# bruAristimunha/Synthetic-Sleep-EEG-Signal-Generation-using-Latent-Diffusion-Models

Hardware: AMD Instinct MI355X
Metric: EEG windows/sec (LDM train step) (higher is better)
Workload: dtype bf16; 1 GPU; LDM train step on raw (B,1,3072) windows: frozen AutoencoderKL[32,32,64] encode+sample x scale, add_noise, config_ldm.yaml UNet (30.5M params, latent_channels=1) fwd+bwd, epsilon MSE, Adam lr 1e-4 [BASELINE configs[2]/[3]: per-GPU batch 256 = global 2048 / 8]; per_gpu_batch=256, global_batch=256, latent_len=768, parallelism=dp1

## Files before the change

### synthetic-sleep-eeg-signal-generation-using-latent-diffusion-models_amd/csrc/gemm.hip

```cpp
#include <stdlib.h>
#include <string.h>

#include "common.h"

namespace {


template <typename T> struct Tr;
template <> struct Tr<float> { static constexpr int KC = 16; static constexpr int EPC = 4; };
template <> struct Tr<bf16_t> { static constexpr int KC = 32; static constexpr int EPC = 8; };
template <> struct Tr<f16_t> { static constexpr int KC = 32; static constexpr int EPC = 8; };

template <typename T> __device__ __forceinline__ void mma(const uint4& a, const uint4& b, f32x4& acc);
template <> __device__ __forceinline__ void mma<float>(const uint4& a, const uint4& b, f32x4& acc) {
  acc = __builtin_amdgcn_mfma_f32_16x16x4f32(__uint_as_float(a.x), __uint_as_float(b.x), acc, 0, 0, 0);
  acc = __builtin_amdgcn_mfma_f32_16x16x4f32(__uint_as_float(a.y), __uint_as_float(b.y), acc, 0, 0, 0);
  acc = __builtin_amdgcn_mfma_f32_16x16x4f32(__uint_as_float(a.z), __uint_as_float(b.z), acc, 0, 0, 0);
  acc = __builtin_amdgcn_mfma_f32_16x16x4f32(__uint_as_float(a.w), __uint_as_float(b.w), acc, 0, 0, 0);
}
template <> __device__ __forceinline__ void mma<bf16_t>(const uint4& a, const uint4& b, f32x4& acc) {
  acc = __builtin_amdgcn_mfma_f32_16x16x32_bf16(__builtin_bit_cast(bf16x8, a), __builtin_bit_cast(bf16x8, b), acc, 0, 0, 0);
}

template <> __device__ __forceinline__ void mma<f16_t>(const uint4& a, const uint4& b, f32x4& acc) {
  acc = __builtin_amdgcn_mfma_f32_16x16x32_f16(__builtin_bit_cast(f16x8, a), __builtin_bit_cast(f16x8, b), acc, 0, 0, 0);
}

typedef s16x4 __attribute__((address_space(3))) * lds_s16x4_ptr;

template <int KSUB> __device__ __forceinline__ int nt_swz(int row, int slot) {
  if constexpr (KSUB == 1) return slot ^ (((row >> 2) & 1) * 3);
  else return slot ^ (2 * ((row >> 1) & 3));
}
template <int BX> __device__ __forceinline__ int tr_swz(int row, int colbyte) {
  constexpr int WIN = ((BX * 2) & (BX * 2 - 1)) == 0 ? BX * 2 - 1 : 127;
  static_assert((BX * 2) % (WIN + 1) == 0, "TR rows must be whole swizzle windows");
  return colbyte ^ ((((row & 3) | (((row >> 3) & 1) << 2)) * 32) & WIN);
}

template <typename T, int BX> struct TrPitch;
template <int BX> struct TrPitch<float, BX> { static constexpr int v = BX * 4 + 16; };
template <int BX> struct TrPitch<bf16_t, BX> { static constexpr int v = BX * 2; };
template <int BX> struct TrPitch<f16_t, BX> { static constexpr int v = BX * 2; };

template <int BX>
__device__ __forceinline__ uint4 read_tr_f32(const char* tile, int ks, int x0, int lm, int q, int rowoff) {
  constexpr int pitch = TrPitch<float, BX>::v;
  const char* p = tile + (ks * 16 + 4 * q + rowoff) * pitch + (x0 + lm) * 4;
  uint4 r;
  r.x = *(const unsigned*)(p);
  r.y = *(const unsigned*)(p + pitch);
  r.z = *(const unsigned*)(p + 2 * pitch);
  r.w = *(const unsigned*)(p + 3 * pitch);
  return r;
}
template <int BX>
__device__ __forceinline__ uint4 read_tr_bf16(const char* tile, int ks, int x0, int lm, int q, int rowoff) {
  constexpr int pitch = TrPitch<bf16_t, BX>::v;
  const int row0 = ks * 32 + 8 * q + (lm >> 2) + rowoff, colb = (x0 + 4 * (lm & 3)) * 2;
  const char* p0 = tile + row0 * pitch + tr_swz<BX>(row0, colb);
  const char* p1 = tile + (row0 + 4) * pitch + tr_swz<BX>(row0 + 4, colb);
  s16x4 lo = __builtin_amdgcn_ds_read_tr16_b64_v4i16((lds_s16x4_ptr)(p0));
  s16x4 hi = __builtin_amdgcn_ds_read_tr16_b64_v4i16((lds_s16x4_ptr)(p1));
  uint4 r;
  r.x = (unsigned)(unsigned short)lo[0] | ((unsigned)(unsigned short)lo[1] << 16);
  r.y = (unsigned)(unsigned short)lo[2] | ((unsigned)(unsigned short)lo[3] << 16);
  r.z = (unsigned)(unsigned short)hi[0] | ((unsigned)(unsigned short)hi[1] << 16);
  r.w = (unsigned)(unsigned short)hi[2] | ((unsigned)(unsigned short)hi[3] << 16);
  return r;
}
template <typename T, int BX>
__device__ __forceinline__ uint4 read_tr_t(const char* tile, int ks, int x0, int lm, int q, int rowoff = 0) {
  if constexpr (sizeof(T) == 4) return read_tr_f32<BX>(tile, ks, x0, lm, q, rowoff);
  else return read_tr_bf16<BX>(tile, ks, x0, lm, q, rowoff);
}
template <typename T, int BX>
__device__ __forceinline__ int tr_store_off(int krow, int seg) {
  if constexpr (sizeof(T) == 4) return krow * TrPitch<float, BX>::v + seg * 16;
  else return krow * TrPitch<bf16_t, BX>::v + tr_swz<BX>(krow, seg * 16);
}

template <typename T, int AMODE, int BMODE, int TAPS, int KSUB, int BN, int STRIDE, int WMT, bool DMA>
struct Cfg {
  static constexpr int WM = (WMT == 3 || WMT == 6) ? 2 : (WMT == 5 ? 4 : WMT);
  static constexpr int FM = (WMT == 3) ? 6 : (WMT == 5 ? 2 : 4);
  static constexpr int BM = WM * FM * 16;
// ... 841 lines not shown
      const float4 v = *(const float4*)(ws + (long)r * n + i);
      s.x += v.x; s.y += v.y; s.z += v.z; s.w += v.w;
    }
  }
  if (ty > 0) red[ty - 1][tx] = s;
  __syncthreads();
  if (ty == 0 && ok) {
    float4 d = *(const float4*)(dst + i);
#pragma unroll
    for (int k = 0; k < 3; k++) { const float4 v = red[k][tx]; s.x += v.x; s.y += v.y; s.z += v.z; s.w += v.w; }
    d.x += s.x; d.y += s.y; d.z += s.z; d.w += s.w;
    *(float4*)(dst + i) = d;
  }
}

__global__ __launch_bounds__(256) void splitk_fold_grouped_kernel(const float* __restrict__ ws, int nsplit, long n, const GemmGroup* __restrict__ grp) {
  __shared__ float4 red[3][64];
  const int tx = threadIdx.x & 63, ty = threadIdx.x >> 6;
  const long i = ((long)blockIdx.x * 64 + tx) * 4;
  const bool ok = i < n;
  const float* w = ws + (long)blockIdx.y * nsplit * n;
  float4 s = make_float4(0.f, 0.f, 0.f, 0.f);
  if (ok) {
    for (int r = ty; r < nsplit; r += 4) {
      const float4 v = *(const float4*)(w + (long)r * n + i);
      s.x += v.x; s.y += v.y; s.z += v.z; s.w += v.w;
    }
  }
  if (ty > 0) red[ty - 1][tx] = s;
  __syncthreads();
  if (ty == 0 && ok) {
    float* dp = grp->Dst[blockIdx.y] + i;
    float4 d = *(const float4*)dp;
#pragma unroll
    for (int k = 0; k < 3; k++) { const float4 v = red[k][tx]; s.x += v.x; s.y += v.y; s.z += v.z; s.w += v.w; }
    d.x += s.x; d.y += s.y; d.z += s.z; d.w += s.w;
    *(float4*)dp = d;
  }
}

int gemm_launch_grouped(eegldm_ctx* ctx, const GemmArgs& a_in, const GemmGroup& g, int slot) {
  GemmArgs a = a_in;
  EEG_CHECK(slot >= 0 && slot < 4096, "group slot");
  if (slot >= ctx->grp_cap) {
    HIP_TRY(hipStreamSynchronize(ctx->stream)); if (ctx->side_on) HIP_TRY(hipStreamSynchronize(ctx->side));
    const int cap = slot + 64;
    GemmGroup* nd = nullptr; HIP_TRY(hipMalloc(&nd, sizeof(GemmGroup) * cap));
    if (ctx->grp_dev) { HIP_TRY(hipMemcpy(nd, ctx->grp_dev, sizeof(GemmGroup) * ctx->grp_cap, hipMemcpyDeviceToDevice)); HIP_TRY(hipFree(ctx->grp_dev)); }
    ctx->grp_dev = nd; ctx->grp_cap = cap; ctx->grp_host.resize(cap);
  }
  if ((int)ctx->grp_host.size() < ctx->grp_cap) ctx->grp_host.resize(ctx->grp_cap);
  if (memcmp(&ctx->grp_host[slot], &g, sizeof(GemmGroup)) != 0) {
    HIP_TRY(hipStreamSynchronize(ctx->stream)); if (ctx->side_on) HIP_TRY(hipStreamSynchronize(ctx->side));
    HIP_TRY(hipMemcpy(ctx->grp_dev + slot, &g, sizeof(GemmGroup), hipMemcpyHostToDevice));
    ctx->grp_host[slot] = g;
  }
  a.grp = ctx->grp_dev + slot;
  EEG_CHECK(a.ngroup >= 1 && a.ngroup <= GEMM_MAX_GROUP && a.amode == GA_TR && a.bmode == GB_TR && a.ztaps == 1 && (a.taps == 1 || a.taps == 3), "not a groupable weight gradient");
  const int epc = a.dtype == EEGLDM_F32 ? 4 : 8;
  EEG_CHECK(a.M % epc == 0 && a.N % epc == 0 && a.N % 4 == 0, "operand alignment");
  for (int i = 0; i < a.ngroup; i++) EEG_CHECK(g.lda[i] % epc == 0 && g.ldb[i] % epc == 0 && g.A[i] && g.B[i] && g.Dst[i], "group member %d: leading dimension / null pointer", i);
  if (a.splitk < 1) a.splitk = 1;
  a.batch = a.ngroup; a.out_f32 = 1; a.ups = 1; a.rows_per_vec = 1; a.ldc = a.N; a.sCt = (long)a.M * a.N; a.colsum = nullptr;
  const long fold_n = (long)a.taps * a.M * a.N;
  const int KST = 2 * (a.dtype == EEGLDM_F32 ? 16 : 32);
  int per = (a.K + a.splitk - 1) / a.splitk; per = (per + KST - 1) / KST * KST;
  a.splitk = (a.K + per - 1) / per;
  const size_t need = (size_t)a.ngroup * a.splitk * fold_n * sizeof(float);
  if (ctx->splitk_ws_bytes < need) {
    if (ctx->splitk_ws) { HIP_TRY(hipStreamSynchronize(ctx->stream)); if (ctx->side_on) HIP_TRY(hipStreamSynchronize(ctx->side)); HIP_TRY(hipFree(ctx->splitk_ws)); ctx->splitk_ws = nullptr; ctx->splitk_ws_bytes = 0; }
    HIP_TRY(hipMalloc(&ctx->splitk_ws, need)); ctx->splitk_ws_bytes = need;
  }
  a.C = ctx->splitk_ws; a.sCk = fold_n; a.sCb = (long)a.splitk * fold_n; a.atomic_out = 0; a.k_skew = 0.f;
  a.zero_page = ctx->zero_page;
  a.xcd_swizzle = 1;
  ProfRec rec; const bool prof = ctx->prof_on;
  if (prof) {
    rec.cls = a.taps == 3 ? PROF_CONV_WGRAD : PROF_GEMM_TN;
    rec.flops = 2.0 * a.M * a.N * (double)a.K * a.taps * a.ngroup;
    rec.M = a.M; rec.N = a.N; rec.K = a.K; rec.taps = a.taps; rec.splitk = a.splitk; rec.kern = "gemm_grouped";
    HIP_TRY(hipEventCreate(&rec.a)); HIP_TRY(hipEventCreate(&rec.b));
    HIP_TRY(hipEventRecord(rec.a, ctx->stream));
  }
  int rc;
  if (a.dtype == EEGLDM_F32) rc = launch_modes<float>(ctx, a);
  else if (a.dtype == EEGLDM_BF16) rc = launch_modes<bf16_t>(ctx, a);
  else if (a.dtype == EEGLDM_F16) rc = launch_modes<f16_t>(ctx, a);
  else EEG_FAIL(EEGLDM_ERR_UNSUPPORTED, "dtype %d", a.dtype);
  if (rc == 0) {
    hipLaunchKernelGGL(splitk_fold_grouped_kernel, dim3((unsigned)((fold_n / 4 + 63) / 64), a.ngroup), dim3(256), 0, ctx->stream, (const float*)ctx->splitk_ws, a.splitk, fold_n, a.grp);
    LAUNCH_CHECK();
  }
  if (prof) { HIP_TRY(hipEventRecord(rec.b, ctx->stream)); ctx->prof.push_back(rec); }
  return rc;
}

int gemm_launch(eegldm_ctx* ctx, const GemmArgs& a_in) {
  GemmArgs a = a_in;
  if (a.splitk < 1) a.splitk = 1;
  if (a.ztaps < 1) a.ztaps = 1;
  if (a.ups < 1) a.ups = 1;
  if (a.batch < 1) a.batch = 1;
  if (a.rows_per_vec < 1) a.rows_per_vec = 1;
  const int epc = a.dtype == EEGLDM_F32 ? 4 : 8;
  EEG_CHECK(a.M > 0 && a.N > 0 && a.K > 0, "empty problem M=%d N=%d K=%d", a.M, a.N, a.K);
  if (a.amode == GA_TR) EEG_CHECK(a.M % epc == 0 && a.lda % epc == 0, "A(TR): M, lda must be multiples of %d", epc);
  else EEG_CHECK(a.K % epc == 0 && a.lda % epc == 0, "A: K, lda must be multiples of %d (K=%d lda=%ld)", epc, a.K, a.lda);
  if (a.bmode == GB_TR) EEG_CHECK(a.N % epc == 0 && a.ldb % epc == 0, "B(TR): N, ldb must be multiples of %d", epc);
  else EEG_CHECK(a.K % epc == 0 && a.ldb % epc == 0, "B: K, ldb must be multiples of %d", epc);
  EEG_CHECK(!(a.atomic_out || a.splitk > 1) || a.out_f32, "atomic / split-K output must be f32");
  EEG_CHECK(a.N % 4 == 0 && a.ldc % 4 == 0, "N and ldc must be multiples of 4 (vector epilogue): N=%d ldc=%ld", a.N, a.ldc);
  EEG_CHECK(!a.resid || a.ldr % 4 == 0, "ldr must be a multiple of 4");
  EEG_CHECK(!a.rowvec || a.ld_rowvec % 4 == 0, "ld_rowvec must be a multiple of 4");
  EEG_CHECK(!a.colsum || (a.amode == GA_TR && a.dtype != EEGLDM_F32 && a.batch == 1), "fused column sums need a 16-bit transposed A operand and batch 1");
  float* fold_dst = nullptr; long fold_n = 0;
  constexpr bool fused_ws = true;
  const bool det_zt = eeg_deterministic() && a.ztaps > 1 && a.taps == 1 && a.sCt == (long)a.M * a.N;
  if (a.splitk > 1 && a.amode == GA_TR && a.bmode == GB_TR && (a.taps == 1 || (a.taps == 3 && a.sCt == (long)a.M * a.N && fused_ws)) && (a.ztaps == 1 || det_zt) && a.batch == 1 && a.atomic_out && a.ldc == a.N) {
    const size_t need = (size_t)a.splitk * a.taps * a.ztaps * a.M * a.N * sizeof(float);
    if (need <= (size_t)512 << 20) {
      if (ctx->splitk_ws_bytes < need) {
        if (ctx->splitk_ws) { HIP_TRY(hipStreamSynchronize(ctx->stream)); HIP_TRY(hipFree(ctx->splitk_ws)); ctx->splitk_ws = nullptr; ctx->splitk_ws_bytes = 0; }
        HIP_TRY(hipMalloc(&ctx->splitk_ws, need)); ctx->splitk_ws_bytes = need;
      }
      const int KST = 2 * (a.dtype == EEGLDM_F32 ? 16 : 32);
      int per = (a.K + a.splitk - 1) / a.splitk; per = (per + KST - 1) / KST * KST;
      a.splitk = (a.K + per - 1) / per;
      fold_dst = (float*)a.C; fold_n = (long)a.taps * a.ztaps * a.M * a.N;
      a.C = ctx->splitk_ws; a.sCk = fold_n; a.atomic_out = 0;
      if (det_zt) HIP_TRY(hipMemsetAsync(ctx->splitk_ws, 0, (size_t)a.splitk * fold_n * sizeof(float), ctx->stream));
    }
  }
  if (a.splitk > 1 && !fold_dst && eeg_deterministic()) a.splitk = 1;
  if (a.splitk > 1 && !fold_dst) a.atomic_out = 1;
  a.zero_page = ctx->zero_page;
  a.xcd_swizzle = 1;
  ProfRec rec; bool prof = ctx->prof_on;
  if (prof) {
    rec.cls = a.amode == GA_CONV ? (a.bmode == GB_NT ? PROF_CONV_FWD : PROF_CONV_DGRAD)
              : (a.amode == GA_TR ? ((a.conv_map || a.taps == 3) ? PROF_CONV_WGRAD : PROF_GEMM_TN) : (a.bmode == GB_NT ? PROF_GEMM_NT : PROF_GEMM_NN));
    rec.flops = 2.0 * a.M * a.N * (double)a.K * a.taps * a.ztaps * a.batch / (a.ups > 1 ? a.ups : 1);
    rec.M = a.M; rec.N = a.N; rec.K = a.K; rec.taps = a.taps * a.ztaps; rec.splitk = a.splitk;
    rec.kern = fold_dst ? "gemm_splitk_fold" : (a.b_kblk ? "gemm_kblk" : "gemm");
    HIP_TRY(hipEventCreate(&rec.a)); HIP_TRY(hipEventCreate(&rec.b));
    HIP_TRY(hipEventRecord(rec.a, ctx->stream));
  }
  a.k_skew = 0.f;
  if (a.splitk > 1 && a.amode == GA_TR && a.atomic_out && !fold_dst) {
    const int kst = (a.dtype == EEGLDM_F32 ? 16 : 32) * 2;
    const long S = ((long)a.K + kst - 1) / kst;
    const float spb = (float)S / (float)a.splitk;
    float sk = (66.0f - spb) / 84.0f;
    sk = sk < 0.f ? 0.f : (sk > 0.5f ? 0.5f : sk);
    if (sk > 0.f && spb * (1.0f - sk) >= 2.0f) a.k_skew = sk;
  }
  int rc = 0;
  if ((a.amode == GA_CONV || (a.amode == GA_PLAIN && a.taps == 1 && a.batch == 1)) && (a.dtype == EEGLDM_BF16 || a.dtype == EEGLDM_F16) && !fold_dst) {
    if (a.bmode == GB_NT) rc = gemm_big_try(ctx, a);
    else if (a.B_alt) { GemmArgs b = a; b.B = a.B_alt; b.bmode = GB_NT; b.b_kblk = 1; rc = gemm_big_try(ctx, b); }
    if (rc < 0) return rc;
  }
  if (rc == 1) { rc = 0; rec.kern = "gemm_big"; }
  else if (a.dtype == EEGLDM_F32) rc = launch_modes<float>(ctx, a);
  else if (a.dtype == EEGLDM_BF16) rc = launch_modes<bf16_t>(ctx, a);
  else if (a.dtype == EEGLDM_F16) rc = launch_modes<f16_t>(ctx, a);
  else EEG_FAIL(EEGLDM_ERR_UNSUPPORTED, "dtype %d", a.dtype);
  if (rc == 0 && fold_dst) {
    hipLaunchKernelGGL(splitk_fold_kernel, dim3((unsigned)((fold_n / 4 + 63) / 64)), dim3(256), 0, ctx->stream, (const float*)ctx->splitk_ws, a.splitk, fold_n, fold_dst);
    LAUNCH_CHECK();
  }
  if (prof) { HIP_TRY(hipEventRecord(rec.b, ctx->stream)); ctx->prof.push_back(rec); }
  return rc;
}
```

### synthetic-sleep-eeg-signal-generation-using-latent-diffusion-models_amd/csrc/internal.h

```cpp
#pragma once
#include "common.h"

int ew_temb(eegldm_ctx*, const int64_t* t, void* out, int B, int dim, int dtype);
int ew_silu(eegldm_ctx*, const float* x, void* y, long n, int dtype);
int ew_silu_bwd(eegldm_ctx*, const float* dy, const float* x, void* dx, long n, int dtype);
int eeg_det_buffer(eegldm_ctx*, size_t bytes, float** out);
int ew_fold_partials_det(eegldm_ctx*, const float* parts, int nparts, long stride, int off, int n, float* total);
int ew_colsum(eegldm_ctx*, const void* x, long ldx, float* out_ps, long ldo, float* total, int B, int L, int C, int dtype);
int ew_softmax(eegldm_ctx*, const float* S, void* P, long rows, int n, int dtype);
int ew_softmax_bwd(eegldm_ctx*, const float* dP, const void* P, void* dS, long rows, int n, float alpha, int dtype);
int ew_add_rows(eegldm_ctx*, void* dst, long ldd, const void* src, long lds, long rows, int C, int dtype);
int ew_dropout_rows(eegldm_ctx*, void* x, long ld, long rows, int C, float p, uint64_t seed, uint64_t offset, int dtype);
int ew_film_silu_fwd(eegldm_ctx*, const void* hn, long ldh, const float* emb, long lde, void* a, long lda, int B, int L, int C, int dtype);
int ew_film_silu_bwd(eegldm_ctx*, const void* hn, long ldh, const float* emb, long lde, const void* da, long ldda, void* dhn, long lddh,
                     float* demb, long ldde, int B, int L, int C, int dtype);
int ew_copy_rows(eegldm_ctx*, void* dst, long ldd, const void* src, long lds, long rows, int C, int dtype);

bool conv_is_thin(int Cin, int Cout, int dtype);
struct KbDesc { long off; long chunk0; int cout, cin; };
int kblk_pack(eegldm_ctx* ctx, const void* w_plain, void* w_packed, const KbDesc* d_table, int n, long total_chunks);
int kblk_pack_one(eegldm_ctx* ctx, const void* w_plain, void* w_packed, int Cout, int Cin, int taps = 3);
int kblk_pack_t(eegldm_ctx* ctx, const void* w_plain, void* w_packed, const KbDesc* d_table, int n, long total_chunks);
int kblk_pack_t_one(eegldm_ctx* ctx, const void* w_plain, void* w_packed, int Cout, int Cin, int taps = 3);
int s2ws_pack(eegldm_ctx* ctx, const void* w, void* wf, void* wd, int Cout, int Cin);
int dconv_run(eegldm_ctx*, int dtype, bool dgrad, const void* in, long ldin, const void* w, const float* bias,
              const void* resid, long ldr, void* out, long ldout, int B, int Lin, int Lout, int Cin, int Cout, int K,
              int stride, int pad_l, float act_slope = 0.f);
bool dconv_fuses_act(int dtype, int Cin, int Cout, int K, long ldout);
int dconv_wgrad(eegldm_ctx*, int dtype, const void* x, long ldx, const void* dy, long lddy, float* dw, int B, int Lin,
                int Lout, int Cin, int Cout, int K, int stride, int pad_l, float* dbias, int* bias_done);
bool dconv_wgrad_tinyv_ok(int Cin, int Cout, int K);

struct SkinnyGn { const float2* part; const float* gamma; const float* beta; int cpg; float eps; int silu;
                  const float2* part_b = nullptr; int nqa = 0; };
struct SkinnyExt { const void* x2; long ldx2; const void* w2; int Cin2; const float* bias2; };
bool conv_skinny_takes(int dtype, int Cin, int Cout, int taps, int B, int L);
int conv_skinny_ex(eegldm_ctx* ctx, int dtype, const void* x, long ldx, const void* w, int Cin, int Cout, int taps, const float* bias,
                   const float* rowvec, long ld_rowvec, const void* resid, long ldr, void* y, long ldy, int B, int L,
                   const SkinnyGn* gn, float2* part_out, const SkinnyExt* ext = nullptr);
int conv_skinny_try(eegldm_ctx* ctx, int dtype, const void* x, long ldx, const void* w, int Cin, int Cout, int taps, const float* bias,
                    const float* rowvec, long ld_rowvec, const void* resid, long ldr, void* y, long ldy, int B, int L);
int conv_ws2_try(eegldm_ctx*, int dtype, int dgrad, const void* x, const void* w, const float* bias, void* y, int B, int Lo,
                 float* col_parts = nullptr, int* col_nparts = nullptr);
int conv_ws_try(eegldm_ctx*, int dtype, const void* x, long ldx, const void* w, int Cin, int Cout, int transposed, const float* bias,
                const float* rowvec, long ld_rowvec, const void* resid, long ldr, void* y, long ldy, int B, int L,
                float* col_parts = nullptr, int* col_nparts = nullptr);

int op_conv_fwd(eegldm_ctx*, int dtype, const void* x, long ldx, const void* w, const float* bias, void* y, long ldy,
                int B, int Lin, int Cin, int Cout, int K, int stride, int pad_l, int pad_r,
                const float* rowvec, long ld_rowvec, const void* resid, long ldr, float act_slope = 0.f,
                float* col_parts = nullptr, int* col_nparts = nullptr);
bool op_conv_fuses_act(int dtype, int Cin, int Cout, int K, long ldy);
int op_conv3_skip_fwd(eegldm_ctx*, int dtype, const void* x, long ldx, const void* w, const float* bias, const void* x2, long ldx2,
                      const void* w2, const float* bias2, void* y, long ldy, int B, int L, int Cin, int Cin2, int Cout,
                      const float* rowvec, long ld_rowvec);
int op_conv_dgrad(eegldm_ctx*, int dtype, const void* dy, long lddy, const void* w, void* dx, long lddx,
                  int B, int Lin, int Cin, int Cout, int K, int stride, int pad_l, int pad_r, const void* resid, long ldr);
bool op_wgrad_fuses_bias(int dtype, int Cin, int Cout);
int op_gn_fold_flush(eegldm_ctx*);
int op_wgrad_flush(eegldm_ctx*);
int op_conv_wgrad(eegldm_ctx*, int dtype, const void* x, long ldx, const void* dy, long lddy, float* dw, float* dbias,
                  int B, int Lin, int Cin, int Cout, int K, int stride, int pad_l, int pad_r);
int op_linear(eegldm_ctx*, int dtype, const void* x, long ldx, const void* w, long ldw, const float* bias, void* y, long ldy,
              int M, int N, int K, int out_f32);
int op_linear_dgrad(eegldm_ctx*, int dtype, const void* dy, long lddy, const void* w, long ldw, void* dx, long lddx,
                    int M, int N, int K, int out_f32);
int op_linear_wgrad(eegldm_ctx*, int dtype, const void* x, long ldx, const void* dy, long lddy, float* dw, long lddw,
                    int M, int N, int K);
int op_attention_fwd(eegldm_ctx*, int dtype, const void* qkv, long ldq, void* out, long ldo, void* probs, float* logits,
                     int B, int T, int C);
int op_attention_bwd(eegldm_ctx*, int dtype, const void* qkv, long ldq, const void* probs, const void* dout, long lddo,
                     void* dqkv, long lddq, float* dprobs, void* dlogits, int B, int T, int C);
int op_groupnorm_bwd(eegldm_ctx*, const void* x, long ldx, const float* gamma, const float* beta, const float* stats,
                     const void* dy, long lddy, void* dx, long lddx, float* dgamma, float* dbeta, int B, int L, int C, int G,
                     int fuse_silu, int resample, const void* dxr, long lddxr, int dtype, float* colsum_ps, long ldps, int* colsum_done,
                     const void* dxr2 = nullptr, long lddxr2 = 0, int* dxr2_done = nullptr, int* slots_deferred = nullptr, int defer_region = 0);
int op_gn_slot_reduce_deferred(eegldm_ctx*, float* dgamma, float* dbeta, int C, int region = 0);
int ew_fold_partials(eegldm_ctx*, const float* parts, int nparts, int n, float* total);
bool pre_conv3_ok(int dtype, int Cin, int Cout, int L);
int pre_conv3_launch(eegldm_ctx*, const void* x, const double* in_stats, const float* gamma, const float* beta, const void* w,
                     const float* bias, const void* resid, void* y, double* out_stats, int B, int L, int Cin, int Cout, float eps, int dtype);
int sample_stats_launch(eegldm_ctx*, const void* x, long n_per_sample, int B, double* stats, int dtype);
bool attn_chain_ok(int dtype, int T, int C, long ldq, long ldo);
int attn_chain_fwd(eegldm_ctx*, const void* qkv, long ldq, void* out, long ldo, void* probs, int B, int T, int C, int dtype);
int attn_chain_bwd(eegldm_ctx*, const void* qkv, long ldq, const void* probs, const void* dout, long lddo, void* dq, long lddq,
                   void* dS, int B, int T, int C, int fuse_kv, int dtype);
bool attn_chain_bwd_fuses_kv(eegldm_ctx*, int B, int T);
```

### synthetic-sleep-eeg-signal-generation-using-latent-diffusion-models_amd/csrc/ops.hip

```cpp
#include <math.h>

#include "common.h"
#include "internal.h"
#include <string.h>

static inline int conv_lout(int Lin, int K, int stride, int pad_l, int pad_r) { return (Lin + pad_l + pad_r - K) / stride + 1; }

bool op_conv_fuses_act(int dtype, int Cin, int Cout, int K, long ldy) { return conv_is_thin(Cin, Cout, dtype) && dconv_fuses_act(dtype, Cin, Cout, K, ldy); }
int op_conv_fwd(eegldm_ctx* ctx, int dtype, const void* x, long ldx, const void* w, const float* bias, void* y, long ldy,
                int B, int Lin, int Cin, int Cout, int K, int stride, int pad_l, int pad_r,
                const float* rowvec, long ld_rowvec, const void* resid, long ldr, float act_slope, float* col_parts, int* col_nparts) {
  if (col_nparts) *col_nparts = 0;
  EEG_CHECK(B > 0 && Lin > 0 && Cin > 0 && Cout > 0 && (K == 1 || K == 3) && (stride == 1 || stride == 2),
            "unsupported conv B=%d Lin=%d Cin=%d Cout=%d K=%d stride=%d", B, Lin, Cin, Cout, K, stride);
  const int Lout = conv_lout(Lin, K, stride, pad_l, pad_r);
  EEG_CHECK(Lout > 0, "empty output");
  if (conv_is_thin(Cin, Cout, dtype)) {
    EEG_CHECK(rowvec == nullptr, "rowvec add is not available on the thin-channel path");
    return dconv_run(ctx, dtype, false, x, ldx, w, bias, resid, ldr, y, ldy, B, Lin, Lout, Cin, Cout, K, stride, pad_l, act_slope);
  }
  EEG_CHECK(act_slope <= 0.f, "fused activation is only available on the thin-input direct conv");
  if (K == 3 && stride == 2 && pad_l == 1 && pad_r == 1 && Cin == 64 && Cout == 128 && ldx == Cin && Lin == 2 * Lout && !rowvec && !resid &&
      dtype != EEGLDM_F32 && !ctx->s2ws_f.empty()) {
    auto it = ctx->s2ws_f.find(w);
// ... 88 lines not shown
    a.amode = GA_CONV; a.tap_flip = 1; a.Lout = Lin; a.Lin = Lin; a.stride = 1; a.pad_l = K - 1 - pad_l;
    a.ups = stride; a.Lsrc = Lout;
    if (dtype != EEGLDM_F32 && stride == 1 && !ctx->kblk_t.empty()) {
      auto it = ctx->kblk_t.find(w);
      if (it != ctx->kblk_t.end()) a.B_alt = it->second;
    }
  }
  return gemm_launch(ctx, a);
}

bool op_wgrad_fuses_bias(int dtype, int Cin, int Cout) {
  EEG_ENV_VAR(bool, fuse_bias, getenv("EEGLDM_NO_FUSED_BIAS_GRAD") == nullptr);
  if (!fuse_bias) return false;
  if (conv_is_thin(Cin, Cout, dtype)) return dconv_wgrad_tinyv_ok(Cin, Cout, 3);
  if (eeg_deterministic()) return false;
  return dtype != EEGLDM_F32;
}

int op_conv_wgrad(eegldm_ctx* ctx, int dtype, const void* x, long ldx, const void* dy, long lddy, float* dw, float* dbias,
                  int B, int Lin, int Cin, int Cout, int K, int stride, int pad_l, int pad_r) {
  const int Lout = conv_lout(Lin, K, stride, pad_l, pad_r);
  const bool thin = conv_is_thin(Cin, Cout, dtype);
  if (thin) {
    EEG_ENV_VAR(bool, fuse_bias, getenv("EEGLDM_NO_FUSED_BIAS_GRAD") == nullptr);
    int done = 0;
    EEG_TRY(dconv_wgrad(ctx, dtype, x, ldx, dy, lddy, dw, B, Lin, Lout, Cin, Cout, K, stride, pad_l, fuse_bias ? dbias : nullptr, &done));
    if (dbias && !done) EEG_TRY(ew_colsum(ctx, dy, lddy, nullptr, 0, dbias, B, Lout, Cout, dtype));
    return 0;
  }
  const bool bias_in_gemm = dbias && op_wgrad_fuses_bias(dtype, Cin, Cout);
  if (dbias && !bias_in_gemm) EEG_TRY(ew_colsum(ctx, dy, lddy, nullptr, 0, dbias, B, Lout, Cout, dtype));
  GemmArgs a = {};
  a.colsum = bias_in_gemm ? dbias : nullptr;
  a.dtype = dtype; a.amode = GA_TR; a.bmode = GB_TR;
  a.A = dy; a.lda = lddy; a.B = x; a.ldb = ldx; a.C = dw; a.ldc = Cin; a.sCt = (long)Cout * Cin;
  a.M = Cout; a.N = Cin; a.K = B * Lout; a.batch = 1; a.taps = 1; a.ztaps = K; a.alpha = 1.0f;
  a.conv_map = !(K == 1 && stride == 1 && pad_l == 0);
  a.Lout = Lout; a.Lin = Lin; a.stride = stride; a.pad_l = pad_l;
  a.out_f32 = 1; a.atomic_out = 1;
  const int kstage = 2 * (dtype == EEGLDM_F32 ? 16 : 32);
  const bool fused3 = (K == 3 && stride == 1 && pad_l == 1 && pad_r == 1 && Lout % kstage == 0);
  int bn = Cin > 64 ? 128 : (Cin > 32 ? 64 : 32);
  long tiles;
  int blocks_per_cu = 2;
  if (fused3) {
    a.taps = 3; a.ztaps = 1; a.conv_map = 0;
    bn = Cin > 32 ? 64 : 32;
    tiles = (long)((Cout + 127) / 128) * ((Cin + bn - 1) / bn);
  } else {
    tiles = (long)((Cout + 127) / 128) * ((Cin + bn - 1) / bn) * K;
  }
  long want = ((long)ctx->num_cu * blocks_per_cu) / tiles;
  long maxs = ((long)a.K + 8 * kstage - 1) / (8 * kstage);
  if (want > maxs) want = maxs;
  a.splitk = (int)(want < 1 ? 1 : want);
  if (ctx->defer_wgrad && (fused3 || (K == 1 && stride == 1 && pad_l == 0 && pad_r == 0)) && a.K % kstage == 0 && !a.wide_n &&
      a.M % 16 == 0 && a.N % 4 == 0) {
    WgradRec r; r.a = a; r.tiles = tiles; r.kstage = kstage; r.dst = dw; r.dbias = bias_in_gemm ? dbias : nullptr;
    r.a.colsum = nullptr; r.a.C = nullptr;
    ctx->wgrad_pending.push_back(r);
    return 0;
  }
  return gemm_launch(ctx, a);
}

int op_wgrad_flush(eegldm_ctx* ctx) {
  std::vector<WgradRec> recs; recs.swap(ctx->wgrad_pending);
  if (recs.empty()) return 0;
  std::vector<char> done(recs.size(), 0);
  const long slots = (long)ctx->num_cu * 2;
  for (size_t i = 0; i < recs.size(); i++) {
    if (done[i]) continue;
    const GemmArgs& k = recs[i].a;
    GemmArgs g = k; g.ngroup = 0;
    GemmGroup tab; memset(&tab, 0, sizeof(tab));
    for (size_t j = i; j < recs.size() && g.ngroup < GEMM_MAX_GROUP; j++) {
      const GemmArgs& o = recs[j].a;
      if (done[j] || o.dtype != k.dtype || o.taps != k.taps || o.ztaps != k.ztaps || o.M != k.M || o.N != k.N || o.K != k.K ||
          o.Lout != k.Lout || o.Lin != k.Lin || o.conv_map != k.conv_map || recs[j].tiles != recs[i].tiles) continue;
      tab.A[g.ngroup] = o.A; tab.B[g.ngroup] = o.B; tab.CS[g.ngroup] = recs[j].dbias; tab.Dst[g.ngroup] = recs[j].dst;
      tab.lda[g.ngroup] = o.lda; tab.ldb[g.ngroup] = o.ldb;
      g.ngroup++; done[j] = 1;
    }
    const long tiles_total = recs[i].tiles * g.ngroup, S = ((long)g.K + recs[i].kstage - 1) / recs[i].kstage;
    long maxs = S / 8; if (maxs < 1) maxs = 1; if (maxs > 256) maxs = 256;
    double best = 1e30; int bs = 1;
    constexpr double c_fixed = 8.0, c_block = 0.05;
    for (long sp = 1; sp <= maxs; sp++) {
      const long blocks = tiles_total * sp, rounds = (blocks + slots - 1) / slots;
      const double cost = (double)rounds * ((double)S / (double)sp + c_fixed) + c_block * (double)blocks;
      if (cost < best) { best = cost; bs = (int)sp; }
    }
    g.splitk = bs; g.batch = g.ngroup;
    EEG_TRY(gemm_launch_grouped(ctx, g, tab, ctx->grp_slot++));
  }
  return 0;
}

int op_linear(eegldm_ctx* ctx, int dtype, const void* x, long ldx, const void* w, long ldw, const float* bias, void* y, long ldy,
              int M, int N, int K, int out_f32) {
  GemmArgs a = {};
  a.dtype = dtype; a.amode = GA_PLAIN; a.bmode = GB_NT; a.A = x; a.lda = ldx; a.B = w; a.ldb = ldw; a.C = y; a.ldc = ldy;
  a.M = M; a.N = N; a.K = K; a.batch = 1; a.taps = 1; a.alpha = 1.0f; a.bias = bias; a.out_f32 = out_f32;
  return gemm_launch(ctx, a);
}
int op_linear_dgrad(eegldm_ctx* ctx, int dtype, const void* dy, long lddy, const void* w, long ldw, void* dx, long lddx,
                    int M, int N, int K, int out_f32) {
  GemmArgs a = {};
  a.dtype = dtype; a.amode = GA_PLAIN; a.bmode = GB_TR; a.A = dy; a.lda = lddy; a.B = w; a.ldb = ldw; a.C = dx; a.ldc = lddx;
  a.M = M; a.N = K; a.K = N; a.batch = 1; a.taps = 1; a.alpha = 1.0f; a.out_f32 = out_f32;
  const long tiles = (long)((M + 127) / 128) * ((K + 127) / 128);
  if (out_f32 && tiles * 8 < ctx->num_cu && N >= 1024) {
    long sk = ctx->num_cu / tiles; const long maxs = N / 256; if (sk > maxs) sk = maxs;
    if (sk > 1) {
      HIP_TRY(hipMemset2DAsync(dx, (size_t)lddx * 4, 0, (size_t)K * 4, M, ctx->stream));
      a.splitk = (int)sk;
    }
  }
  return gemm_launch(ctx, a);
}
int op_linear_wgrad(eegldm_ctx* ctx, int dtype, const void* x, long ldx, const void* dy, long lddy, float* dw, long lddw,
                    int M, int N, int K) {
  GemmArgs a = {};
  a.dtype = dtype; a.amode = GA_TR; a.bmode = GB_TR; a.A = dy; a.lda = lddy; a.B = x; a.ldb = ldx; a.C = dw; a.ldc = lddw;
  a.M = N; a.N = K; a.K = M; a.batch = 1; a.taps = 1; a.alpha = 1.0f; a.out_f32 = 1; a.atomic_out = 1;
  return gemm_launch(ctx, a);
}

int op_attention_fwd(eegldm_ctx* ctx, int dtype, const void* qkv, long ldq, void* out, long ldo, void* probs, float* logits,
                     int B, int T, int C) {
  if (attn_chain_ok(dtype, T, C, ldq, ldo)) return attn_chain_fwd(ctx, qkv, ldq, out, ldo, probs, B, T, C, dtype);
  const size_t es = dtype_size(dtype);
  const char* q = (const char*)qkv; const char* k = q + (size_t)C * es; const char* v = q + (size_t)2 * C * es;
  GemmArgs a = {};
  a.dtype = dtype; a.amode = GA_PLAIN; a.bmode = GB_NT; a.A = q; a.lda = ldq; a.sAb = (long)T * ldq; a.B = k; a.ldb = ldq;
  a.sBb = (long)T * ldq; a.C = logits; a.ldc = T; a.sCb = (long)T * T; a.M = T; a.N = T; a.K = C; a.batch = B; a.taps = 1;
  a.alpha = 1.0f / sqrtf((float)C);
  a.out_f32 = 1;
  EEG_TRY(gemm_launch(ctx, a));
  EEG_TRY(ew_softmax(ctx, logits, probs, (long)B * T, T, dtype));
  GemmArgs b = {};
  b.dtype = dtype; b.amode = GA_PLAIN; b.bmode = GB_TR; b.A = probs; b.lda = T; b.sAb = (long)T * T; b.B = v; b.ldb = ldq;
  b.sBb = (long)T * ldq; b.C = out; b.ldc = ldo; b.sCb = (long)T * ldo; b.M = T; b.N = C; b.K = T; b.batch = B; b.taps = 1;
  b.alpha = 1.0f;
  return gemm_launch(ctx, b);
}

int op_attention_bwd(eegldm_ctx* ctx, int dtype, const void* qkv, long ldq, const void* probs, const void* dout, long lddo,
                     void* dqkv, long lddq, float* dprobs, void* dlogits, int B, int T, int C) {
  const size_t es = dtype_size(dtype);
  const char* q = (const char*)qkv; const char* k = q + (size_t)C * es; const char* v = q + (size_t)2 * C * es;
  char* dq = (char*)dqkv; char* dk = dq + (size_t)C * es; char* dv = dq + (size_t)2 * C * es;
  const float alpha = 1.0f / sqrtf((float)C);
  GemmArgs g = {};
  const bool fused = attn_chain_ok(dtype, T, C, ldq, lddo) && lddq % 8 == 0;
  EEG_ENV_VAR(bool, no_fused_v, getenv("EEGLDM_ATTN_NO_FUSED_DV") != nullptr);
  const int fk = (fused && attn_chain_bwd_fuses_kv(ctx, B, T)) ? (no_fused_v ? 1 : 2) : 0;
  if (fk != 2) {
  g.dtype = dtype; g.amode = GA_TR; g.bmode = GB_TR; g.A = probs; g.lda = T; g.sAb = (long)T * T; g.B = dout; g.ldb = lddo;
  g.sBb = (long)T * lddo; g.C = dv; g.ldc = lddq; g.sCb = (long)T * lddq; g.M = T; g.N = C; g.K = T; g.batch = B; g.taps = 1; g.alpha = 1.f;
  EEG_TRY(gemm_launch(ctx, g));
  }
  if (fused) {
    EEG_TRY(attn_chain_bwd(ctx, qkv, ldq, probs, dout, lddo, dq, lddq, dlogits, B, T, C, fk, dtype));
    if (fk) return 0;
  } else {
  g = GemmArgs{};
  g.dtype = dtype; g.amode = GA_PLAIN; g.bmode = GB_NT; g.A = dout; g.lda = lddo; g.sAb = (long)T * lddo; g.B = v; g.ldb = ldq;
  g.sBb = (long)T * ldq; g.C = dprobs; g.ldc = T; g.sCb = (long)T * T; g.M = T; g.N = T; g.K = C; g.batch = B; g.taps = 1; g.alpha = 1.f;
  g.out_f32 = 1;
  EEG_TRY(gemm_launch(ctx, g));
  EEG_TRY(ew_softmax_bwd(ctx, dprobs, probs, dlogits, (long)B * T, T, alpha, dtype));
// ... 125 lines not shown
```

Baseline: 14450 windows/s.

## Add persistent 128x128 LDS-ring wgrad kernel for 3-tap conv weight gradients

Adds a new persistent, warp-specialized bf16/f16 weight-gradient kernel for 3-tap convolutions. It uses 128x128x64 tiles, a 4-stage LDS ring filled by global_load_lds DMA, transposed LDS reads, XCD-aware unit distribution, and fused column-sum via MFMA with ones. Both the grouped and single wgrad launch paths now try this kernel first, and the split-k cost model counts tiles and slots for the bigger tile. The aim is better data reuse and overlap on large conv wgrad GEMMs. The risks are eligibility gaps, register pressure, and hand-tuned waitcnt correctness.

```diff
diff --git a/synthetic-sleep-eeg-signal-generation-using-latent-diffusion-models_amd/csrc/gemm.hip b/synthetic-sleep-eeg-signal-generation-using-latent-diffusion-models_amd/csrc/gemm.hip
--- a/synthetic-sleep-eeg-signal-generation-using-latent-diffusion-models_amd/csrc/gemm.hip
+++ b/synthetic-sleep-eeg-signal-generation-using-latent-diffusion-models_amd/csrc/gemm.hip
@@ -2,6 +2,7 @@
 #include <string.h>
 
 #include "common.h"
+#include "internal.h"
 
 namespace {
 
@@ -1009,8 +1010,10 @@
     HIP_TRY(hipEventCreate(&rec.a)); HIP_TRY(hipEventCreate(&rec.b));
     HIP_TRY(hipEventRecord(rec.a, ctx->stream));
   }
-  int rc;
-  if (a.dtype == EEGLDM_F32) rc = launch_modes<float>(ctx, a);
+  int rc = a.taps == 3 ? wgrad_big_try(ctx, a) : 0;
+  if (rc < 0) return rc;
+  if (rc == 1) rc = 0;
+  else if (a.dtype == EEGLDM_F32) rc = launch_modes<float>(ctx, a);
   else if (a.dtype == EEGLDM_BF16) rc = launch_modes<bf16_t>(ctx, a);
   else if (a.dtype == EEGLDM_F16) rc = launch_modes<f16_t>(ctx, a);
   else EEG_FAIL(EEGLDM_ERR_UNSUPPORTED, "dtype %d", a.dtype);
@@ -1088,6 +1091,7 @@
     if (rc < 0) return rc;
   }
   if (rc == 1) { rc = 0; rec.kern = "gemm_big"; }
+  else if (fold_dst && a.taps == 3 && (rc = wgrad_big_try(ctx, a)) != 0) { if (rc < 0) return rc; rc = 0; }
   else if (a.dtype == EEGLDM_F32) rc = launch_modes<float>(ctx, a);
   else if (a.dtype == EEGLDM_BF16) rc = launch_modes<bf16_t>(ctx, a);
   else if (a.dtype == EEGLDM_F16) rc = launch_modes<f16_t>(ctx, a);
diff --git a/synthetic-sleep-eeg-signal-generation-using-latent-diffusion-models_amd/csrc/internal.h b/synthetic-sleep-eeg-signal-generation-using-latent-diffusion-models_amd/csrc/internal.h
--- a/synthetic-sleep-eeg-signal-generation-using-latent-diffusion-models_amd/csrc/internal.h
+++ b/synthetic-sleep-eeg-signal-generation-using-latent-diffusion-models_amd/csrc/internal.h
@@ -86,3 +86,7 @@
 int attn_chain_bwd(eegldm_ctx*, const void* qkv, long ldq, const void* probs, const void* dout, long lddo, void* dq, long lddq,
                    void* dS, int B, int T, int C, int fuse_kv, int dtype);
 bool attn_chain_bwd_fuses_kv(eegldm_ctx*, int B, int T);
+
+bool wgrad_big_eligible(const GemmArgs& a);
+int wgrad_big_grid(const eegldm_ctx* ctx);
+int wgrad_big_try(eegldm_ctx* ctx, const GemmArgs& a);
diff --git a/synthetic-sleep-eeg-signal-generation-using-latent-diffusion-models_amd/csrc/ops.hip b/synthetic-sleep-eeg-signal-generation-using-latent-diffusion-models_amd/csrc/ops.hip
--- a/synthetic-sleep-eeg-signal-generation-using-latent-diffusion-models_amd/csrc/ops.hip
+++ b/synthetic-sleep-eeg-signal-generation-using-latent-diffusion-models_amd/csrc/ops.hip
@@ -194,12 +194,14 @@
       tab.lda[g.ngroup] = o.lda; tab.ldb[g.ngroup] = o.ldb;
       g.ngroup++; done[j] = 1;
     }
-    const long tiles_total = recs[i].tiles * g.ngroup, S = ((long)g.K + recs[i].kstage - 1) / recs[i].kstage;
+    const bool big = wgrad_big_eligible(g);
+    const long unit_tiles = big ? (long)(g.M / 128) * (g.N / 128) : recs[i].tiles, unit_slots = big ? wgrad_big_grid(ctx) : slots;
+    const long tiles_total = unit_tiles * g.ngroup, S = ((long)g.K + recs[i].kstage - 1) / recs[i].kstage;
     long maxs = S / 8; if (maxs < 1) maxs = 1; if (maxs > 256) maxs = 256;
     double best = 1e30; int bs = 1;
     constexpr double c_fixed = 8.0, c_block = 0.05;
     for (long sp = 1; sp <= maxs; sp++) {
-      const long blocks = tiles_total * sp, rounds = (blocks + slots - 1) / slots;
+      const long blocks = tiles_total * sp, rounds = (blocks + unit_slots - 1) / unit_slots;
       const double cost = (double)rounds * ((double)S / (double)sp + c_fixed) + c_block * (double)blocks;
       if (cost < best) { best = cost; bs = (int)sp; }
     }
diff --git a/synthetic-sleep-eeg-signal-generation-using-latent-diffusion-models_amd/csrc/wgrad_big.hip b/synthetic-sleep-eeg-signal-generation-using-latent-diffusion-models_amd/csrc/wgrad_big.hip
--- /dev/null
+++ b/synthetic-sleep-eeg-signal-generation-using-latent-diffusion-models_amd/csrc/wgrad_big.hip
@@ -0,0 +1,325 @@
+#include <stdlib.h>
+
+#include <type_traits>
+
+#include "common.h"
+#include "internal.h"
+
+namespace {
+
+constexpr int WB_BM = 128, WB_BN = 128, WB_BK = 64, WB_NTHR = 512, WB_NLOAD = 4;
+constexpr int WB_FM = 4, WB_FN = 2;
+constexpr int WB_PITCH = 256;
+constexpr int WB_A_BYTES = WB_BK * WB_PITCH;
+constexpr int WB_B_ALLOC = 17 * 1024;
+constexpr int WB_STAGE = WB_A_BYTES + WB_B_ALLOC;
+constexpr int WB_NSTG = 4;
+constexpr int WB_LDS = WB_NSTG * WB_STAGE;
+constexpr int WB_NST = 3 * WB_FM * 4 * WB_FN;
+constexpr int WB_LDS_TOTAL = WB_LDS + (int)sizeof(GemmGroup);
+static_assert(WB_LDS_TOTAL <= 160 * 1024 && sizeof(GemmGroup) % 16 == 0, "ring does not fit the 160 KiB LDS");
+
+typedef __attribute__((address_space(3))) void* wb_lds_ptr;
+typedef s16x4 __attribute__((address_space(3))) * wb_lds_s16x4_ptr;
+
+struct WgArgs {
+  const void* A; long lda;
+  const void* B; long ldb;
+  float* colsum;
+  const GemmGroup* grp;
+  float* C; long sCb, sCk, sCt, ldc;
+  int M, N, K, L;
+  int splitk, per;
+  int tiles_n, tiles, units, ngroup;
+  float alpha;
+  const void* zero_page;
+};
+
+__device__ __forceinline__ int wb_swz(int row, int colbyte) { return colbyte ^ ((((row & 3) | (((row >> 3) & 1) << 2)) * 32) & 255); }
+
+__device__ __forceinline__ void wb_dma(const void* g, unsigned lds_off) {
+  asm volatile("s_mov_b32 m0, %0\n\ts_nop 0\n\tglobal_load_lds_dwordx4 %1, off" ::"s"(__builtin_amdgcn_readfirstlane(lds_off)), "v"(g) : "memory", "m0");
+}
+__device__ __forceinline__ void wb_dmas(const void* base, unsigned voff, unsigned lds_off) {
+  const unsigned long long u = (unsigned long long)base;
+  const unsigned lo = __builtin_amdgcn_readfirstlane((unsigned)u), hi = __builtin_amdgcn_readfirstlane((unsigned)(u >> 32));
+  const unsigned long long b = ((unsigned long long)hi << 32) | lo;
+  asm volatile("s_mov_b32 m0, %0\n\ts_nop 0\n\tglobal_load_lds_dwordx4 %1, %2" ::"s"(__builtin_amdgcn_readfirstlane(lds_off)), "v"(voff), "s"(b) : "memory", "m0");
+}
+__device__ __forceinline__ const void* wb_uniform(const void* ptr) {
+  const unsigned long long u = (unsigned long long)ptr;
+  const unsigned lo = __builtin_amdgcn_readfirstlane((unsigned)u), hi = __builtin_amdgcn_readfirstlane((unsigned)(u >> 32));
+  return (const void*)(((unsigned long long)hi << 32) | lo);
+}
+template <typename T> __device__ __forceinline__ f32x4 wb_mma(const uint4& a, const uint4& b, const f32x4& c) {
+  if constexpr (Is16<T>::f16) return __builtin_amdgcn_mfma_f32_16x16x32_f16(__builtin_bit_cast(f16x8, a), __builtin_bit_cast(f16x8, b), c, 0, 0, 0);
+  else return __builtin_amdgcn_mfma_f32_16x16x32_bf16(__builtin_bit_cast(bf16x8, a), __builtin_bit_cast(bf16x8, b), c, 0, 0, 0);
+}
+__device__ __forceinline__ uint4 wb_frag(const char* base, unsigned o0, unsigned o1) {
+  const s16x4 lo = __builtin_amdgcn_ds_read_tr16_b64_v4i16((wb_lds_s16x4_ptr)(base + o0));
+  const s16x4 hi = __builtin_amdgcn_ds_read_tr16_b64_v4i16((wb_lds_s16x4_ptr)(base + o1));
+  uint4 r;
+  r.x = (unsigned)(unsigned short)lo[0] | ((unsigned)(unsigned short)lo[1] << 16);
+  r.y = (unsigned)(unsigned short)lo[2] | ((unsigned)(unsigned short)lo[3] << 16);
+  r.z = (unsigned)(unsigned short)hi[0] | ((unsigned)(unsigned short)hi[1] << 16);
+  r.w = (unsigned)(unsigned short)hi[2] | ((unsigned)(unsigned short)hi[3] << 16);
+  return r;
+}
+__device__ __forceinline__ void wb_frag_off(int rowoff, int x0, int lm, int q, unsigned& o0, unsigned& o1) {
+  const int row0 = 8 * q + (lm >> 2) + rowoff, colb = (x0 + 4 * (lm & 3)) * 2;
+  o0 = (unsigned)(row0 * WB_PITCH + wb_swz(row0, colb));
+  o1 = (unsigned)((row0 + 4) * WB_PITCH + wb_swz(row0 + 4, colb));
+}
+
+template <typename T>
+__global__ __launch_bounds__(WB_NTHR, 1) void wgrad_big_kernel(const WgArgs p) {
+  extern __shared__ __attribute__((aligned(16))) char smem[];
+  const int tid = threadIdx.x, lane = tid & 63, wave = tid >> 6;
+  const int lm = lane & 15, q = lane >> 4;
+  const int wm = wave >> 2, wn = wave & 3;
+  const unsigned wave_u = __builtin_amdgcn_readfirstlane(wave);
+  const unsigned lds0 = (unsigned)(size_t)(wb_lds_ptr)smem;
+
+  const int nwx = (int)gridDim.x >> 3, xcd = (int)blockIdx.x & 7, wl = (int)blockIdx.x >> 3;
+  const int q8 = p.units >> 3, r8 = p.units & 7;
+  const int run0 = xcd * q8 + min(xcd, r8), runn = q8 + (xcd < r8 ? 1 : 0);
+  auto unit_of = [&](int j) -> int { const int i = wl + j * nwx; return i < runn ? run0 + i : -1; };
+  struct Unit { int bz, sp, m0, n0, kbeg, nst; };
+  auto decode = [&](int u, Unit& d) __attribute__((always_inline)) {
+    const int tile = u % p.tiles, rest = u / p.tiles;
+    d.sp = rest % p.splitk; d.bz = rest / p.splitk;
+    d.m0 = (tile / p.tiles_n) * WB_BM; d.n0 = (tile % p.tiles_n) * WB_BN;
+    d.kbeg = d.sp * p.per;
+    d.nst = (min(p.K, d.kbeg + p.per) - d.kbeg) / WB_BK;
+  };
+  if (unit_of(0) < 0) return;
+  GemmGroup* const tab = (GemmGroup*)(smem + WB_LDS);
+  if (p.ngroup) {
+    for (int i = tid; i < (int)(sizeof(GemmGroup) / 8); i += WB_NTHR) ((unsigned long long*)tab)[i] = ((const unsigned long long*)p.grp)[i];
+  } else if (tid == 0) {
+    tab->A[0] = p.A; tab->B[0] = p.B; tab->CS[0] = p.colsum; tab->lda[0] = p.lda; tab->ldb[0] = p.ldb;
+  }
+  __syncthreads();
+
+  unsigned aoff[WB_FM][2], boff[3][WB_FN][2];
+#pragma unroll
+  for (int i = 0; i < WB_FM; i++) wb_frag_off(0, wm * 64 + i * 16, lm, q, aoff[i][0], aoff[i][1]);
+#pragma unroll
+  for (int t = 0; t < 3; t++)
+#pragma unroll
+    for (int j = 0; j < WB_FN; j++) wb_frag_off(t, wn * 32 + j * 16, lm, q, boff[t][j][0], boff[t][j][1]);
+
+  auto run = [&](auto loader_tag) __attribute__((always_inline)) {
+    constexpr bool LOADER = decltype(loader_tag)::value;
+    const int r4 = lane >> 4;
+    const int seg = (lane & 15) ^ ((r4 | (((int)(wave_u >> 1) & 1) << 2)) * 2);
+    const T* zeros = (const T*)p.zero_page;
+    int ij = 0; Unit iu; bool ivalid = false; int is = 0;
+    const T* iA = nullptr; const T* iB = nullptr; long ilda = 0, ildb = 0; unsigned a_voff = 0, b_voff = 0;
+    auto iset = [&]() __attribute__((always_inline)) {
+      const int u = unit_of(ij);
+      ivalid = u >= 0; is = 0;
+      if (!ivalid) return;
+      decode(u, iu);
+      iA = (const T*)wb_uniform(tab->A[iu.bz]); iB = (const T*)wb_uniform(tab->B[iu.bz]);
+      ilda = (long)wb_uniform((const void*)tab->lda[iu.bz]); ildb = (long)wb_uniform((const void*)tab->ldb[iu.bz]);
+      a_voff = (unsigned)(((long)r4 * ilda + seg * 8) * 2);
+      b_voff = (unsigned)(((long)r4 * ildb + seg * 8) * 2);
+    };
+    const T* acur = nullptr; const T* bcur = nullptr; const T* h0 = nullptr; const T* h1 = nullptr;
+    unsigned idst = 0;
+    auto begin_stage = [&](int buf) __attribute__((always_inline)) {
+      const int k0 = iu.kbeg + is * WB_BK;
+      acur = (const T*)wb_uniform(iA + (long)(k0 + 4 * (int)wave_u) * ilda + iu.m0);
+      bcur = (const T*)wb_uniform(iB + (long)(k0 - 1 + 4 * (int)wave_u) * ildb + iu.n0);
+      idst = lds0 + (unsigned)(buf * WB_STAGE);
+      if (wave_u == 0) {
+        const bool top_ok = k0 % p.L != 0, bot_ok = (k0 + WB_BK) % p.L != 0;
+        const T* col = iB + iu.n0 + seg * 8;
+        h0 = (r4 > 0 || top_ok) ? col + (long)(k0 - 1 + r4) * ildb : zeros;
+        h1 = (r4 == 0 || (r4 == 1 && bot_ok)) ? col + (long)(k0 + 63 + r4) * ildb : zeros;
+      }
+    };
+    auto issue = [&](int k) __attribute__((always_inline)) {
+      if (k < 4) {
+        wb_dmas(acur, a_voff, idst + (wave_u + 4 * k) * 1024u);
+        acur += 16 * ilda;
+      } else if (k < 8) {
+        const unsigned d = idst + WB_A_BYTES + (wave_u + 4 * (k - 4)) * 1024u;
+        if (k == 4 && wave_u == 0) wb_dma(h0, d);
+        else wb_dmas(bcur, b_voff, d);
+        bcur += 16 * ildb;
+      } else if (wave_u == 0) {
+        wb_dma(h1, idst + WB_A_BYTES + 16 * 1024u);
+      }
+    };
+    auto advance = [&]() __attribute__((always_inline)) { if (++is == iu.nst) { ij++; iset(); } };
+    int inflight = 0;
+    if constexpr (LOADER) {
+      iset();
+#pragma unroll 1
+      for (int g = 0; g < WB_NSTG - 1 && ivalid; g++) {
+        begin_stage(g);
+#pragma unroll
+        for (int k = 0; k < 9; k++) issue(k);
+        advance();
+        inflight++;
+      }
+    }
+
+    int cj = 0; Unit cu; decode(unit_of(0), cu); int cs_ = 0;
+    float* csum = nullptr;
+    auto cset = [&]() __attribute__((always_inline)) {
+      float* const c = (float*)wb_uniform(tab->CS[cu.bz]);
+      csum = (cu.n0 == 0 && (wave_u & 3) == 0) ? c : nullptr;
+    };
+    cset();
+    f32x4 acc[3][WB_FM][WB_FN];
+    f32x4 cs[WB_FM];
+    auto zero_acc = [&]() __attribute__((always_inline)) {
+#pragma unroll
+      for (int t = 0; t < 3; t++)
+#pragma unroll
+        for (int i = 0; i < WB_FM; i++)
+#pragma unroll
+          for (int j = 0; j < WB_FN; j++) acc[t][i][j] = f32x4{0.f, 0.f, 0.f, 0.f};
+#pragma unroll
+      for (int i = 0; i < WB_FM; i++) cs[i] = f32x4{0.f, 0.f, 0.f, 0.f};
+    };
+    zero_acc();
+    int last_store = -8;
+#pragma unroll 1
+    for (int g = 0;; g++) {
+      if constexpr (LOADER) {
+        const int after = min(2, inflight - 1);
+        if (g <= last_store + 3) asm volatile("s_waitcnt vmcnt(63)" ::: "memory");
+        else if (after >= 2) { if (wave_u == 0) asm volatile("s_waitcnt vmcnt(18)" ::: "memory"); else asm volatile("s_waitcnt vmcnt(16)" ::: "memory"); }
+        else if (after == 1) { if (wave_u == 0) asm volatile("s_waitcnt vmcnt(9)" ::: "memory"); else asm volatile("s_waitcnt vmcnt(8)" ::: "memory"); }
+        else asm volatile("s_waitcnt vmcnt(0)" ::: "memory");
+      }
+      __builtin_amdgcn_s_barrier();
+      asm volatile("" ::: "memory");
+      bool do_issue = false;
+      if constexpr (LOADER) {
+        do_issue = ivalid;
+        if (do_issue) begin_stage((g + WB_NSTG - 1) % WB_NSTG);
+      }
+      const char* sb = smem + (g % WB_NSTG) * WB_STAGE;
+      const char* sa1 = sb + 32 * WB_PITCH;
+      const char* sbB = sb + WB_A_BYTES;
+      uint4 af[2][WB_FM], bf[2][WB_FN];
+      auto load = [&](int st) __attribute__((always_inline)) {
+        const int ks = st / 3, t = st % 3;
+        if (t == 0) {
+#pragma unroll
+          for (int i = 0; i < WB_FM; i++) af[ks][i] = wb_frag(ks ? sa1 : sb, aoff[i][0], aoff[i][1]);
+        }
+#pragma unroll
+        for (int j = 0; j < WB_FN; j++) bf[st & 1][j] = wb_frag(sbB + ks * 32 * WB_PITCH, boff[t][j][0], boff[t][j][1]);
+      };
+      load(0);
+      __builtin_amdgcn_sched_barrier(0);
+#pragma unroll
+      for (int st = 0; st < 6; st++) {
+        if (st + 1 < 6) load(st + 1);
+        __builtin_amdgcn_sched_barrier(0);
+        const int ks = st / 3, t = st % 3;
+#pragma unroll
+        for (int i = 0; i < WB_FM; i++)
+#pragma unroll
+          for (int j = 0; j < WB_FN; j++) {
+            acc[t][i][j] = wb_mma<T>(af[ks][i], bf[st & 1][j], acc[t][i][j]);
+            if constexpr (LOADER) {
+              const int m = st * (WB_FM * WB_FN) + i * WB_FN + j;
+              if (m >= 1 && (m - 1) % 5 == 0 && (m - 1) / 5 < 9 && do_issue) {
+                __builtin_amdgcn_sched_barrier(0);
+                issue((m - 1) / 5);
+                __builtin_amdgcn_sched_barrier(0);
+              }
+            }
+          }
+      }
+      if (csum) {
+        constexpr unsigned ONE2 = Is16<T>::f16 ? 0x3C003C00u : 0x3F803F80u;
+        const uint4 ones = make_uint4(ONE2, ONE2, ONE2, ONE2);
+#pragma unroll
+        for (int ks = 0; ks < 2; ks++)
+#pragma unroll
+          for (int i = 0; i < WB_FM; i++) cs[i] = wb_mma<T>(af[ks][i], ones, cs[i]);
+      }
+      if constexpr (LOADER) {
+        if (do_issue) { advance(); inflight++; }
+        inflight--;
+      }
+      if (++cs_ == cu.nst) {
+        float* cp = p.C + (long)cu.bz * p.sCb + (long)cu.sp * p.sCk;
+#pragma unroll
+        for (int t = 0; t < 3; t++)
+#pragma unroll
+          for (int i = 0; i < WB_FM; i++)
+#pragma unroll
+            for (int r = 0; r < 4; r++) {
+              const int m = cu.m0 + wm * 64 + i * 16 + q * 4 + r;
+#pragma unroll
+              for (int j = 0; j < WB_FN; j++) cp[(long)t * p.sCt + (long)m * p.ldc + cu.n0 + wn * 32 + j * 16 + lm] = acc[t][i][j][r] * p.alpha;
+            }
+        if (csum && lm == 0) {
+#pragma unroll
+          for (int i = 0; i < WB_FM; i++)
+#pragma unroll
+            for (int r = 0; r < 4; r++) atomicAdd(csum + cu.m0 + wm * 64 + i * 16 + q * 4 + r, cs[i][r]);
+        }
+        last_store = g;
+        zero_acc();
+        const int u = unit_of(++cj);
+        if (u < 0) return;
+        decode(u, cu); cs_ = 0;
+        cset();
+      }
+    }
+  };
+  if (wave_u < WB_NLOAD) run(std::true_type{}); else run(std::false_type{});
+}
+
+}
+
+bool wgrad_big_eligible(const GemmArgs& a) {
+  EEG_ENV_VAR(bool, off, getenv("EEGLDM_NO_WGRAD_BIG") != nullptr);
+  if (off) return false;
+  return (a.dtype == EEGLDM_BF16 || a.dtype == EEGLDM_F16) && a.amode == GA_TR && a.bmode == GB_TR && a.taps == 3 && a.ztaps <= 1 &&
+         !a.conv_map && a.M % WB_BM == 0 && a.N % WB_BN == 0 && a.Lout > 0 && a.Lout % WB_BK == 0 && a.K % a.Lout == 0 &&
+         a.K % WB_BK == 0 && a.sCt == (long)a.M * a.N && a.ldc == a.N;
+}
+
+int wgrad_big_grid(const eegldm_ctx* ctx) { const int g = (ctx->num_cu / 8) * 8; return g < 8 ? 8 : g; }
+
+int wgrad_big_try(eegldm_ctx* ctx, const GemmArgs& a) {
+  if (!wgrad_big_eligible(a) || a.sCk != 3L * a.M * a.N || a.atomic_out || (a.batch != 1 && !a.ngroup)) return 0;
+  WgArgs w = {};
+  w.A = a.A; w.lda = a.lda; w.B = a.B; w.ldb = a.ldb; w.colsum = a.ngroup ? nullptr : a.colsum; w.grp = a.ngroup ? a.grp : nullptr;
+  w.C = (float*)a.C; w.sCb = a.ngroup ? a.sCb : 0; w.sCk = a.sCk; w.sCt = a.sCt; w.ldc = a.ldc;
+  w.M = a.M; w.N = a.N; w.K = a.K; w.L = a.Lout;
+  w.splitk = a.splitk < 1 ? 1 : a.splitk;
+  int per = (a.K + w.splitk - 1) / w.splitk; per = (per + WB_BK - 1) / WB_BK * WB_BK;
+  EEG_CHECK((a.K + per - 1) / per == w.splitk, "wgrad_big: split count %d leaves empty splits (K = %d)", w.splitk, a.K);
+  w.per = per;
+  w.tiles_n = a.N / WB_BN; w.tiles = (a.M / WB_BM) * w.tiles_n;
+  w.ngroup = a.ngroup;
+  const long units = (long)w.tiles * w.splitk * (a.ngroup ? a.ngroup : 1);
+  EEG_CHECK(units < (1L << 30), "wgrad_big: too many units");
+  w.units = (int)units;
+  w.alpha = a.alpha; w.zero_page = ctx->zero_page;
+  if (!a.ngroup) EEG_CHECK(a.lda % 8 == 0 && a.ldb % 8 == 0, "wgrad_big: leading dimensions");
+  long grid = wgrad_big_grid(ctx);
+  const long need = (units + 7) / 8 * 8;
+  if (need < grid) grid = need;
+  auto launch = [&](auto kern) -> int {
+    static DevOnce once;
+    if (once.need(ctx->device)) HIP_TRY(hipFuncSetAttribute((const void*)kern, hipFuncAttributeMaxDynamicSharedMemorySize, WB_LDS_TOTAL));
+    hipLaunchKernelGGL(kern, dim3((unsigned)grid), dim3(WB_NTHR), WB_LDS_TOTAL, ctx->stream, w);
+    LAUNCH_CHECK();
+    return 1;
+  };
+  if (a.dtype == EEGLDM_F16) return launch(wgrad_big_kernel<f16_t>);
+  return launch(wgrad_big_kernel<bf16_t>);
+}
```

Result: faster. 14650 windows/s (median of 6 runs) (+1.4%).
